# lawfuyang/ToyRenderer

Hardware: AMD Instinct MI355X
Metric: Gmeshlets/s culled (whole node), 100M meshlets (higher is better)
Workload: dtype f32

## Files before the change

### include/trhip.h

```cpp
#ifndef TRHIP_H_
#define TRHIP_H_

#include <stddef.h>
#include <stdint.h>

#ifdef __cplusplus
extern "C" {
#endif

#define TRHIP_ABI_VERSION 1

typedef struct trhip_device_t*  trhip_device;
typedef struct trhip_heap_t*    trhip_heap;
typedef struct trhip_buffer_t*  trhip_buffer;
typedef struct trhip_texture_t* trhip_texture;
typedef struct trhip_cmdlist_t* trhip_cmdlist;
typedef struct trhip_timer_t*   trhip_timer;
typedef struct trhip_pipeline_stats_t* trhip_pipeline_stats;

enum {
    TRHIP_OK = 0,
    TRHIP_ERR_INVALID = -1,
    TRHIP_ERR_HIP = -2,
    TRHIP_ERR_UNKNOWN_SHADER = -3,
    TRHIP_ERR_STATE = -4,
    TRHIP_ERR_NO_DEVICE = -5
};

enum { TRHIP_FORMAT_R16_FLOAT = 1, TRHIP_FORMAT_R32_FLOAT = 2, TRHIP_FORMAT_RG32_UINT = 3, TRHIP_FORMAT_RG16_FLOAT = 4,
       TRHIP_FORMAT_RGBA32_UINT = 5, TRHIP_FORMAT_R11G11B10_FLOAT = 6, TRHIP_FORMAT_R8_UNORM = 7, TRHIP_FORMAT_R8_UINT = 8 };

const char* trhip_last_error(void);
uint32_t    trhip_abi_version(void);
uint32_t    trhip_shader_count(void);
const char* trhip_shader_name(uint32_t index);
int         trhip_shader_exists(const char* name);

int  trhip_device_create(int device_index, trhip_device* out);
int  trhip_device_create_on_stream(int device_index, void* hip_stream, trhip_device* out);
void trhip_device_destroy(trhip_device dev);
int  trhip_device_wait_idle(trhip_device dev);
int  trhip_device_join_side_stream(trhip_device dev);
int  trhip_device_info(trhip_device dev, uint32_t* compute_units, uint32_t* wave_size, uint64_t* total_mem);
void* trhip_device_stream(trhip_device dev);

typedef struct {
    uint64_t    byteSize;
    uint32_t    structStride;
    uint32_t    canHaveUAVs;
    uint32_t    isDrawIndirectArgs;
    uint32_t    isVirtual;
    uint32_t    isVolatileConstant;
    const char* debugName;
} trhip_buffer_desc;

typedef struct {
    uint32_t    width, height, mipLevels;
    uint32_t    format;
    uint32_t    isUAV;
    uint32_t    isVirtual;
    const char* debugName;
} trhip_texture_desc;

int  trhip_heap_create(trhip_device dev, uint64_t bytes, trhip_heap* out);
void trhip_heap_release(trhip_heap heap);

int  trhip_buffer_create(trhip_device dev, const trhip_buffer_desc* desc, trhip_buffer* out);
int  trhip_buffer_wrap(trhip_device dev, void* device_ptr, const trhip_buffer_desc* desc, trhip_buffer* out);
int  trhip_buffer_memory_requirements(trhip_buffer buf, uint64_t* size, uint64_t* alignment);
int  trhip_buffer_bind_memory(trhip_buffer buf, trhip_heap heap, uint64_t offset);
void trhip_buffer_retain(trhip_buffer buf);
void trhip_buffer_release(trhip_buffer buf);
void* trhip_buffer_device_ptr(trhip_buffer buf);
uint64_t trhip_buffer_size(trhip_buffer buf);

int  trhip_texture_create(trhip_device dev, const trhip_texture_desc* desc, trhip_texture* out);
int  trhip_texture_memory_requirements(trhip_texture tex, uint64_t* size, uint64_t* alignment);
int  trhip_texture_bind_memory(trhip_texture tex, trhip_heap heap, uint64_t offset);
void trhip_texture_retain(trhip_texture tex);
void trhip_texture_release(trhip_texture tex);
void* trhip_texture_device_ptr(trhip_texture tex);
int  trhip_texture_mip_info(trhip_texture tex, uint32_t mip, uint32_t* w, uint32_t* h, uint64_t* byte_offset);
uint64_t trhip_texture_size(trhip_texture tex);

int  trhip_buffer_upload(trhip_buffer buf, uint64_t dst_offset, const void* src, uint64_t bytes);
int  trhip_buffer_download(trhip_buffer buf, uint64_t src_offset, void* dst, uint64_t bytes);
int  trhip_texture_upload(trhip_texture tex, uint32_t mip, const void* src, uint64_t bytes);
int  trhip_texture_download(trhip_texture tex, uint32_t mip, void* dst, uint64_t bytes);

int  trhip_buffer_mark_written(trhip_buffer buf);
int  trhip_texture_mark_written(trhip_texture tex);

typedef enum {
    TRHIP_BIND_CONSTANT_BUFFER = 0,
    TRHIP_BIND_PUSH_CONSTANTS  = 1,
    TRHIP_BIND_STRUCTURED_SRV  = 2,
    TRHIP_BIND_STRUCTURED_UAV  = 3,
    TRHIP_BIND_TEXTURE_SRV     = 4,
    TRHIP_BIND_TEXTURE_UAV     = 5,
    TRHIP_BIND_SAMPLER         = 6
} trhip_binding_type;

typedef struct {
    uint32_t type;
    uint32_t slot;
    void*    resource;
    uint32_t baseMip;
    uint32_t reserved;
} trhip_binding;

int  trhip_cmd_create(trhip_device dev, trhip_cmdlist* out);
void trhip_cmd_release(trhip_cmdlist cl);
int  trhip_cmd_open(trhip_cmdlist cl);
int  trhip_cmd_close(trhip_cmdlist cl);
int  trhip_cmd_write_buffer(trhip_cmdlist cl, trhip_buffer buf, uint64_t dst_offset, const void* src, uint64_t bytes);
int  trhip_cmd_clear_buffer_u32(trhip_cmdlist cl, trhip_buffer buf, uint32_t value);
int  trhip_cmd_clear_texture_f32(trhip_cmdlist cl, trhip_texture tex, float value);
int  trhip_cmd_clear_texture_u32(trhip_cmdlist cl, trhip_texture tex, uint32_t value);
int  trhip_cmd_copy_buffer(trhip_cmdlist cl, trhip_buffer dst, uint64_t dst_offset, trhip_buffer src, uint64_t src_offset, uint64_t bytes);
typedef void (*trhip_host_fn)(void* user, void* hip_stream);
int  trhip_cmd_host_callback(trhip_cmdlist cl, trhip_host_fn fn, void* user);
int  trhip_cmd_copy_texture(trhip_cmdlist cl, trhip_texture dst, trhip_texture src);
int  trhip_cmd_dispatch(trhip_cmdlist cl, const char* shader_name,
                        const trhip_binding* bindings, uint32_t num_bindings,
                        const void* push_constants, uint32_t push_bytes,
                        uint32_t gx, uint32_t gy, uint32_t gz);
int  trhip_cmd_dispatch_indirect(trhip_cmdlist cl, const char* shader_name,
                                 const trhip_binding* bindings, uint32_t num_bindings,
                                 const void* push_constants, uint32_t push_bytes,
                                 trhip_buffer args_buffer, uint32_t args_offset_bytes);
int  trhip_cmd_begin_timer(trhip_cmdlist cl, trhip_timer t);
int  trhip_cmd_end_timer(trhip_cmdlist cl, trhip_timer t);
int  trhip_cmd_begin_marker(trhip_cmdlist cl, const char* name);
int  trhip_cmd_end_marker(trhip_cmdlist cl);

int  trhip_queue_execute(trhip_device dev, const trhip_cmdlist* lists, uint32_t num_lists);

int  trhip_timer_create(trhip_device dev, trhip_timer* out);
void trhip_timer_release(trhip_timer t);
int  trhip_timer_get_ms(trhip_timer t, float* ms);

typedef struct {
    uint64_t IAVertices, IAPrimitives, VSInvocations, GSInvocations, GSPrimitives, CInvocations, CPrimitives, PSInvocations,
             HSInvocations, DSInvocations, CSInvocations, ASInvocations, MSInvocations, MSPrimitives;
} trhip_pipeline_statistics;

int  trhip_pipeline_stats_create(trhip_device dev, trhip_pipeline_stats* out);
void trhip_pipeline_stats_release(trhip_pipeline_stats q);
int  trhip_cmd_begin_pipeline_stats(trhip_cmdlist cl, trhip_pipeline_stats q);
int  trhip_cmd_end_pipeline_stats(trhip_cmdlist cl, trhip_pipeline_stats q);
int  trhip_pipeline_stats_get(trhip_pipeline_stats q, trhip_pipeline_statistics* out);

int  trhip_profile_enable(trhip_device dev, int enabled);
int  trhip_profile_filter(trhip_device dev, const char* name);
int  trhip_profile_reset(trhip_device dev);
int  trhip_profile_count(trhip_device dev, uint32_t* n);
int  trhip_profile_entry(trhip_device dev, uint32_t index, const char** name, uint64_t* launches, double* total_ms);

int  trhip_stream_create(int device_index, void** out_hip_stream);
int  trhip_stream_create_priority(int device_index, int priority_class, void** out_hip_stream);
void trhip_stream_destroy(void* hip_stream);
int  trhip_stream_synchronize(void* hip_stream);
int  trhip_event_create(int device_index, void** out_hip_event);
void trhip_event_destroy(void* hip_event);
int  trhip_event_record(void* hip_event, void* hip_stream);
int  trhip_stream_wait_event(void* hip_stream, void* hip_event);

int  trhip_launch_shard_late_info(void* hip_stream, const uint32_t* gathered_counts, uint32_t world, uint32_t rank, uint32_t* info);

#ifdef __cplusplus
}
#endif
#endif
```

### toyrenderer_amd/csrc/k_hzb.hip

```cpp
#include "cull_math.hip.h"
#include "hzb_quad.hip.h"
#include "trhip_internal.h"

using namespace interop;

namespace
{

template <bool MAX>
__global__ __launch_bounds__(256) void minMaxDownsampleKernel(const float* __restrict__ depth, uint32_t W, uint32_t H,
                                                              _Float16* __restrict__ out, uint32_t ow, uint32_t oh)
{
    const uint32_t x = blockIdx.x * 32 + (threadIdx.x & 31), y = blockIdx.y * 8 + (threadIdx.x >> 5);
    if (x >= ow || y >= oh) return;
    const float u = ((float)x + 0.5f) / (float)ow, v = ((float)y + 0.5f) / (float)oh;
    const float fx = cm::fma_(u, (float)W, -0.5f), fy = cm::fma_(v, (float)H, -0.5f);
    int x0 = (int)__builtin_floorf(fx), y0 = (int)__builtin_floorf(fy);
    int x1 = min(max(x0 + 1, 0), (int)W - 1), y1 = min(max(y0 + 1, 0), (int)H - 1);
    x0 = min(max(x0, 0), (int)W - 1);
    y0 = min(max(y0, 0), (int)H - 1);
    const float a = depth[(uint64_t)y0 * W + x0], b = depth[(uint64_t)y0 * W + x1];
    const float c = depth[(uint64_t)y1 * W + x0], d = depth[(uint64_t)y1 * W + x1];
    const float r = MAX ? cm::max_(cm::max_(a, b), cm::max_(c, d))
                        : cm::min_(cm::min_(a, b), cm::min_(c, d));
    out[(uint64_t)y * ow + x] = (_Float16)r;
}

struct SpdArgs
{
    _Float16* base;
    uint32_t width, height, mips;
    uint32_t mipOffset[16];
};

template <bool MAX>
__device__ __forceinline__ float red4(float a, float b, float c, float d)
{
    return MAX ? cm::max_(cm::max_(a, b), cm::max_(c, d)) : cm::min_(cm::min_(a, b), cm::min_(c, d));
}

template <bool MAX>
__global__ __launch_bounds__(256) void spdTileKernel(SpdArgs a, uint32_t lastMip)
{
    __shared__ float s[2][32 * 32];
    const uint32_t tid = threadIdx.x;
    const uint32_t tx = blockIdx.x, ty = blockIdx.y;
    const _Float16* m0 = a.base + a.mipOffset[0];
    {
        const uint32_t px = (tid & 15) * 2, py = (tid >> 4) * 2;
        for (uint32_t dy = 0; dy < 2; ++dy)
            for (uint32_t dx = 0; dx < 2; ++dx) {
                const uint32_t ox = px + dx, oy = py + dy;
                const uint32_t sx = tx * 64 + ox * 2, sy = ty * 64 + oy * 2;
                const float v = red4<MAX>((float)m0[(uint64_t)sy * a.width + sx], (float)m0[(uint64_t)sy * a.width + sx + 1],
                                          (float)m0[(uint64_t)(sy + 1) * a.width + sx], (float)m0[(uint64_t)(sy + 1) * a.width + sx + 1]);
                s[0][oy * 32 + ox] = v;
                if (lastMip >= 1) {
                    const uint32_t mw = a.width >> 1;
                    a.base[a.mipOffset[1] + (uint64_t)(ty * 32 + oy) * mw + tx * 32 + ox] = (_Float16)v;
                }
            }
    }
    __syncthreads();
    uint32_t cur = 0, dim = 32;
    for (uint32_t mip = 2; mip <= 6 && mip <= lastMip; ++mip) {
        const uint32_t od = dim >> 1;
        if (tid < od * od) {
            const uint32_t ox = tid % od, oy = tid / od;
            const float* p = s[cur];
            const float v = red4<MAX>(p[(2 * oy) * dim + 2 * ox], p[(2 * oy) * dim + 2 * ox + 1],
                                      p[(2 * oy + 1) * dim + 2 * ox], p[(2 * oy + 1) * dim + 2 * ox + 1]);
            s[cur ^ 1][oy * od + ox] = v;
            const uint32_t mw = a.width >> mip;
            a.base[a.mipOffset[mip] + (uint64_t)(ty * od + oy) * mw + tx * od + ox] = (_Float16)v;
        }
        __syncthreads();
        cur ^= 1;
        dim = od;
    }
}

template <bool MAX>
__global__ __launch_bounds__(256) void hzbDepthTileKernel(const float* __restrict__ depth, uint32_t W, uint32_t H, SpdArgs a, uint32_t lastMip)
{
    __shared__ float s0[64 * 64];
    __shared__ float s[2][32 * 32];
    const uint32_t tid = threadIdx.x;
    const uint32_t tx = blockIdx.x, ty = blockIdx.y;
    _Float16* m0 = a.base + a.mipOffset[0];
    const uint32_t ow = a.width, oh = a.height;
    {
        const uint32_t lx = tid & 63u, x = tx * 64 + lx;
        const float u = ((float)x + 0.5f) / (float)ow;
        const float fx = cm::fma_(u, (float)W, -0.5f);
        int x0 = (int)__builtin_floorf(fx);
        const int x1 = min(max(x0 + 1, 0), (int)W - 1);
        x0 = min(max(x0, 0), (int)W - 1);
        const int xl = min(x0, (int)W - 2);
        struct __attribute__((packed, aligned(4))) Pair { float a, b; };
        const bool wide = W >= 2u;
        Pair v0[16], v1[16];
        int rowY0, rowY1;
        {
            const uint32_t ly = (tid & 15u) * 4 + (tid >> 6), y = ty * 64 + ly;
            const float v = ((float)y + 0.5f) / (float)oh;
            const float fy = cm::fma_(v, (float)H, -0.5f);
            const int f0 = (int)__builtin_floorf(fy);
            rowY1 = min(max(f0 + 1, 0), (int)H - 1);
            rowY0 = min(max(f0, 0), (int)H - 1);
        }
#pragma unroll
        for (uint32_t it = 0; it < 16; ++it) {
            const int y0 = __builtin_amdgcn_readlane(rowY0, (int)it), y1 = __builtin_amdgcn_readlane(rowY1, (int)it);
            if (wide) {
                v0[it] = *reinterpret_cast<const Pair*>(depth + (uint64_t)y0 * W + xl);
                v1[it] = *reinterpret_cast<const Pair*>(depth + (uint64_t)y1 * W + xl);
            } else {
                v0[it] = { depth[(uint64_t)y0 * W + x0], depth[(uint64_t)y0 * W + x1] };
                v1[it] = { depth[(uint64_t)y1 * W + x0], depth[(uint64_t)y1 * W + x1] };
            }
        }
#pragma unroll
        for (uint32_t it = 0; it < 16; ++it) {
            const uint32_t ly = it * 4 + (tid >> 6), y = ty * 64 + ly;
            const float p = !wide || x0 == xl ? v0[it].a : v0[it].b, q = wide && x1 == xl ? v0[it].a : v0[it].b;
            const float r = !wide || x0 == xl ? v1[it].a : v1[it].b, t = wide && x1 == xl ? v1[it].a : v1[it].b;
            const _Float16 h = (_Float16)red4<MAX>(p, q, r, t);
            m0[(uint64_t)y * ow + x] = h;
            s0[ly * 64 + lx] = (float)h;
        }
    }
    __syncthreads();
    {
        const uint32_t px = (tid & 15) * 2, py = (tid >> 4) * 2;
        for (uint32_t dy = 0; dy < 2; ++dy)
            for (uint32_t dx = 0; dx < 2; ++dx) {
                const uint32_t ox = px + dx, oy = py + dy;
                const float v = red4<MAX>(s0[(2 * oy) * 64 + 2 * ox], s0[(2 * oy) * 64 + 2 * ox + 1],
                                          s0[(2 * oy + 1) * 64 + 2 * ox], s0[(2 * oy + 1) * 64 + 2 * ox + 1]);
                s[0][oy * 32 + ox] = v;
                if (lastMip >= 1) {
                    const uint32_t mw = a.width >> 1;
                    a.base[a.mipOffset[1] + (uint64_t)(ty * 32 + oy) * mw + tx * 32 + ox] = (_Float16)v;
                }
            }
    }
    __syncthreads();
    uint32_t cur = 0, dim = 32;
    for (uint32_t mip = 2; mip <= 6 && mip <= lastMip; ++mip) {
        const uint32_t od = dim >> 1;
        if (tid < od * od) {
            const uint32_t ox = tid % od, oy = tid / od;
            const float* p = s[cur];
            const float v = red4<MAX>(p[(2 * oy) * dim + 2 * ox], p[(2 * oy) * dim + 2 * ox + 1],
                                      p[(2 * oy + 1) * dim + 2 * ox], p[(2 * oy + 1) * dim + 2 * ox + 1]);
            s[cur ^ 1][oy * od + ox] = v;
            const uint32_t mw = a.width >> mip;
            a.base[a.mipOffset[mip] + (uint64_t)(ty * od + oy) * mw + tx * od + ox] = (_Float16)v;
        }
        __syncthreads();
        cur ^= 1;
        dim = od;
    }
}

template <bool MAX>
__global__ __launch_bounds__(256) void spdMipKernel(SpdArgs a, uint32_t mip)
{
    const uint32_t pw = (a.width >> (mip - 1)) ? (a.width >> (mip - 1)) : 1u, ph = (a.height >> (mip - 1)) ? (a.height >> (mip - 1)) : 1u;
    const uint32_t mw = (a.width >> mip) ? (a.width >> mip) : 1u, mh = (a.height >> mip) ? (a.height >> mip) : 1u;
    const uint32_t i = blockIdx.x * 256u + threadIdx.x;
    if (i >= mw * mh) return;
    const uint32_t x = i % mw, y = i / mw;
    const uint32_t x0 = min(2 * x, pw - 1), x1 = min(2 * x + 1, pw - 1);
    const uint32_t y0 = min(2 * y, ph - 1), y1 = min(2 * y + 1, ph - 1);
    const _Float16* p = a.base + a.mipOffset[mip - 1];
    a.base[a.mipOffset[mip] + i] = (_Float16)red4<MAX>((float)p[y0 * pw + x0], (float)p[y0 * pw + x1], (float)p[y1 * pw + x0], (float)p[y1 * pw + x1]);
}

struct MinMaxNote { const float* depth; uint32_t W, H; _Float16* out; uint32_t ow, oh; bool mx; };

template <bool MAX>
__global__ __launch_bounds__(1024) void spdTailKernel(SpdArgs a, uint32_t first)
{
    __shared__ float s[2][64 * 64];
    const uint32_t tid = threadIdx.x;
    uint32_t pw = (a.width >> first) ? (a.width >> first) : 1u, ph = (a.height >> first) ? (a.height >> first) : 1u;
    for (uint32_t i = tid; i < pw * ph; i += 1024) s[0][i] = (float)a.base[a.mipOffset[first] + i];
    __syncthreads();
    uint32_t cur = 0;
    for (uint32_t mip = first + 1; mip < a.mips; ++mip) {
        const uint32_t mw = (a.width >> mip) ? (a.width >> mip) : 1u, mh = (a.height >> mip) ? (a.height >> mip) : 1u;
        const float* p = s[cur];
        for (uint32_t i = tid; i < mw * mh; i += 1024) {
            const uint32_t x = i % mw, y = i / mw;
            const uint32_t x0 = min(2 * x, pw - 1), x1 = min(2 * x + 1, pw - 1);
            const uint32_t y0 = min(2 * y, ph - 1), y1 = min(2 * y + 1, ph - 1);
            const float v = red4<MAX>(p[y0 * pw + x0], p[y0 * pw + x1], p[y1 * pw + x0], p[y1 * pw + x1]);
            s[cur ^ 1][i] = v;
            a.base[a.mipOffset[mip] + i] = (_Float16)v;
        }
        __syncthreads();
        cur ^= 1;
        pw = mw; ph = mh;
    }
}

__global__ __launch_bounds__(256) void hzbQuadBuildKernel(trhip::QuadArgs a)
{
    __shared__ float s_t[9][trhip::kQuadStripCols + 1];
    trhip::hzbQuadStrip(a, blockIdx.x, s_t);
}


int recordMinMaxDownsample(trhip::DispatchCtx& ctx)
{
    const MinMaxDownsampleConsts* k = (const MinMaxDownsampleConsts*)ctx.constants(0, sizeof(MinMaxDownsampleConsts));
    TRHIP_REQUIRE(k, "%s: push constants (MinMaxDownsampleConsts, 12 bytes) missing", ctx.shaderName);
    trhip_texture_t* src = ctx.texture(TRHIP_BIND_TEXTURE_SRV, 0);
    uint32_t mip = 0;
    trhip_texture_t* dst = ctx.texture(TRHIP_BIND_TEXTURE_UAV, 0, &mip);
    TRHIP_REQUIRE(src && dst, "%s: needs Texture_SRV t0 (depth) and Texture_UAV u0 (HZB)", ctx.shaderName);
    TRHIP_REQUIRE(src->format == TRHIP_FORMAT_R32_FLOAT, "%s: depth source must be R32_FLOAT", ctx.shaderName);
    TRHIP_REQUIRE(dst->format == TRHIP_FORMAT_R16_FLOAT, "%s: HZB must be R16_FLOAT", ctx.shaderName);
    TRHIP_REQUIRE(k->m_OutputDimensions.x == dst->mipW(mip) && k->m_OutputDimensions.y == dst->mipH(mip),
                  "%s: m_OutputDimensions %ux%u does not match HZB mip %u (%ux%u)", ctx.shaderName,
                  k->m_OutputDimensions.x, k->m_OutputDimensions.y, mip, dst->mipW(mip), dst->mipH(mip));
    TRHIP_REQUIRE(!ctx.indirect, "%s: dispatched directly", ctx.shaderName);
    TRHIP_REQUIRE(ctx.gx >= (dst->mipW(mip) + 7) / 8 && ctx.gy >= (dst->mipH(mip) + 7) / 8,
                  "%s: dispatch %ux%u groups of 8x8 does not cover %ux%u (BasePassRenderers.cpp:533)", ctx.shaderName,
                  ctx.gx, ctx.gy, dst->mipW(mip), dst->mipH(mip));
    const float* depth = (const float*)src->mipPtr(0);
    _Float16* out = (_Float16*)dst->mipPtr(mip);
    const uint32_t W = src->width, H = src->height, ow = dst->mipW(mip), oh = dst->mipH(mip);
    const bool mx = k->m_bDownsampleMax != 0;
    ctx.emit("main", [=](hipStream_t s) {
        dim3 grid((ow + 31) / 32, (oh + 7) / 8);
        if (mx) TRHIP_LAUNCH(minMaxDownsampleKernel<true>, grid, dim3(256), 0, s, depth, W, H, out, ow, oh);
        else TRHIP_LAUNCH(minMaxDownsampleKernel<false>, grid, dim3(256), 0, s, depth, W, H, out, ow, oh);
        return trhip::launchStatus("minMaxDownsampleKernel"); });
    ctx.cl->peephole = { ctx.cl->ops.size() - 1, "minmaxdownsample", std::make_shared<MinMaxNote>(MinMaxNote{ depth, W, H, out, ow, oh, mx }) };
    return TRHIP_OK;
}

int recordSPD(trhip::DispatchCtx& ctx)
{
    const SPDConstants* k = (const SPDConstants*)ctx.constants(0, sizeof(SPDConstants));
    TRHIP_REQUIRE(k, "%s: push constants (SPDConstants, 32 bytes) missing", ctx.shaderName);
    uint32_t mip0 = 0;
    trhip_texture_t* tex = ctx.texture(TRHIP_BIND_TEXTURE_UAV, 2, &mip0);
    TRHIP_REQUIRE(tex, "%s: needs Texture_UAV u2 = HZB mip 0 (FFXHelpers.cpp:71)", ctx.shaderName);
    TRHIP_REQUIRE(mip0 == 0, "%s: u2 must be mip 0", ctx.shaderName);
    TRHIP_REQUIRE(tex->format == TRHIP_FORMAT_R16_FLOAT, "%s: HZB must be R16_FLOAT", ctx.shaderName);
    TRHIP_REQUIRE(k->mips == tex->mips - 1, "%s: SPDConstants.mips %u != HZB mips-1 %u (FFXHelpers.cpp:63-64)", ctx.shaderName, k->mips, tex->mips - 1);
    for (uint32_t i = 1; i < tex->mips; ++i) {
        uint32_t m = 0;
        trhip_texture_t* t = ctx.texture(TRHIP_BIND_TEXTURE_UAV, 2 + i, &m);
        TRHIP_REQUIRE(t == tex && m == i, "%s: UAV u%u must be HZB mip %u (FFXHelpers.cpp:76-81)", ctx.shaderName, 2 + i, i);
    }
    TRHIP_REQUIRE(!ctx.indirect, "%s: dispatched directly", ctx.shaderName);
    if (trhip_buffer_t* counter = ctx.buffer(TRHIP_BIND_STRUCTURED_UAV, 0)) ctx.cl->forgetUse(counter->ptr, ctx.cl->ops.size());
    const bool mx = ctx.variant == 2;
    SpdArgs a;
    memset(&a, 0, sizeof a);
    a.base = (_Float16*)tex->ptr;
    a.width = tex->width; a.height = tex->height; a.mips = tex->mips;
    for (uint32_t i = 0; i < tex->mips; ++i) a.mipOffset[i] = (uint32_t)(tex->mipOffset[i] / 2);
    if (tex->mips <= 1) return TRHIP_OK;

    uint32_t first = 0;
    const bool tiled = (tex->width % 64 == 0) && (tex->height % 64 == 0);
    const trhip_cmdlist_t::Peephole ph = ctx.cl->peephole;
    const MinMaxNote* note = (ph.kind && !strcmp(ph.kind, "minmaxdownsample") && ph.op == ctx.cl->ops.size() - 1 && ph.op != SIZE_MAX) ? (const MinMaxNote*)ph.data.get() : nullptr;
    const bool fuse = tiled && note && note->out == a.base + a.mipOffset[0] && note->ow == tex->width && note->oh == tex->height && note->mx == mx
                      && ctx.cl->ops.back().lane == 0;
    if (fuse) {
        const MinMaxNote n = *note;
        const uint32_t lastMip = tex->mips - 1 < 6 ? tex->mips - 1 : 6;
        ctx.cl->ops.pop_back();
        ctx.emit("depth_tile", [a, n, lastMip, mx](hipStream_t s) {
            dim3 grid(a.width / 64, a.height / 64);
            if (mx) TRHIP_LAUNCH(hzbDepthTileKernel<true>, grid, dim3(256), 0, s, n.depth, n.W, n.H, a, lastMip);
            else TRHIP_LAUNCH(hzbDepthTileKernel<false>, grid, dim3(256), 0, s, n.depth, n.W, n.H, a, lastMip);
            return trhip::launchStatus("hzbDepthTileKernel"); });
        first = lastMip;
    } else if (tiled) {
        const uint32_t lastMip = tex->mips - 1 < 6 ? tex->mips - 1 : 6;
        ctx.emit("tile", [a, lastMip, mx](hipStream_t s) {
            dim3 grid(a.width / 64, a.height / 64);
            if (mx) TRHIP_LAUNCH(spdTileKernel<true>, grid, dim3(256), 0, s, a, lastMip);
            else TRHIP_LAUNCH(spdTileKernel<false>, grid, dim3(256), 0, s, a, lastMip);
            return trhip::launchStatus("spdTileKernel"); });
        first = lastMip;
    }
    while ((uint64_t)tex->mipW(first) * tex->mipH(first) > 64 * 64 && first + 1 < tex->mips) {
        const uint32_t mip = first + 1;
        const uint32_t texels = tex->mipW(mip) * tex->mipH(mip);
        ctx.emit("mip", [a, mip, texels, mx](hipStream_t s) {
            if (mx) TRHIP_LAUNCH(spdMipKernel<true>, dim3((texels + 255u) / 256u), dim3(256), 0, s, a, mip);
            else TRHIP_LAUNCH(spdMipKernel<false>, dim3((texels + 255u) / 256u), dim3(256), 0, s, a, mip);
            return trhip::launchStatus("spdMipKernel"); });
        first = mip;
    }
    if (first + 1 < tex->mips) {
        ctx.emit("tail", [a, first, mx](hipStream_t s) {
            if (mx) TRHIP_LAUNCH(spdTailKernel<true>, dim3(1), dim3(1024), 0, s, a, first);
            else TRHIP_LAUNCH(spdTailKernel<false>, dim3(1), dim3(1024), 0, s, a, first);
            return trhip::launchStatus("spdTailKernel"); });
    }
    return TRHIP_OK;
}

}

namespace trhip
{

int hzbQuadEnsure(trhip_texture_t* tex)
{
    TRHIP_REQUIRE(tex && tex->ptr && tex->format == TRHIP_FORMAT_R16_FLOAT && tex->mips <= 16, "footprint-min table: needs a bound R16_FLOAT texture");
    uint64_t total = 0;
    for (uint32_t k = 0; k < tex->mips; ++k) {
        tex->quadOffset[k] = (uint32_t)total;
        total += (uint64_t)((tex->mipW(k) >> 3) + 1) * ((tex->mipH(k) >> 3) + 1) * 64u;
    }
    TRHIP_REQUIRE(total < (1ull << 31), "footprint-min table: HZB %ux%u too large", tex->width, tex->height);
    tex->quadTotal = (uint32_t)total;
    return tex->quad.allocate(tex->dev, total * 2);
}

int hzbQuadLaunchBuild(trhip_texture_t* tex, hipStream_t s)
{
    const Stamp from = { tex->version };
    if (tex->quad.current(from)) return TRHIP_OK;
    const QuadArgs a = quadArgs(tex);
    TRHIP_LAUNCH(hzbQuadBuildKernel, dim3(a.firstStrip[a.mips]), dim3(256), 0, s, a);
    tex->quad.markBuilt(from);
    return launchStatus("hzbQuadBuildKernel");
}

}

namespace
{

trhip::ShaderRegistrar r0("minmaxdownsample_CS_Main", recordMinMaxDownsample, 0);
trhip::ShaderRegistrar r1("ffx_spd_downsample_pass_CS FFX_SPD_OPTION_DOWNSAMPLE_FILTER=1", recordSPD, 1);
trhip::ShaderRegistrar r2("ffx_spd_downsample_pass_CS FFX_SPD_OPTION_DOWNSAMPLE_FILTER=2", recordSPD, 2);

}
```

### toyrenderer_amd/rhi.py

```python
from __future__ import annotations

import ctypes as C
import os

import numpy as np

_HERE = os.path.dirname(os.path.abspath(__file__))
LIB_PATH = os.environ.get("TRHIP_LIB") or os.path.join(_HERE, "lib", "libtrhip.so")

FORMAT_R16_FLOAT = 1
FORMAT_R32_FLOAT = 2
FORMAT_RG32_UINT = 3
FORMAT_RG16_FLOAT = 4
FORMAT_RGBA32_UINT = 5
FORMAT_R11G11B10_FLOAT = 6
FORMAT_R8_UNORM = 7
FORMAT_R8_UINT = 8

BIND_CONSTANT_BUFFER, BIND_PUSH_CONSTANTS, BIND_STRUCTURED_SRV, BIND_STRUCTURED_UAV, BIND_TEXTURE_SRV, BIND_TEXTURE_UAV, BIND_SAMPLER = range(7)

ABI_SYMBOLS = [
    "trhip_last_error", "trhip_abi_version", "trhip_shader_count", "trhip_shader_name", "trhip_shader_exists",
    "trhip_device_create", "trhip_device_create_on_stream", "trhip_device_destroy", "trhip_device_wait_idle",
    "trhip_device_info", "trhip_device_stream", "trhip_device_join_side_stream",
    "trhip_heap_create", "trhip_heap_release",
    "trhip_buffer_create", "trhip_buffer_wrap", "trhip_buffer_memory_requirements", "trhip_buffer_bind_memory",
    "trhip_buffer_retain", "trhip_buffer_release", "trhip_buffer_device_ptr", "trhip_buffer_size",
    "trhip_texture_create", "trhip_texture_memory_requirements", "trhip_texture_bind_memory", "trhip_texture_retain",
    "trhip_texture_release", "trhip_texture_device_ptr", "trhip_texture_mip_info", "trhip_texture_size",
    "trhip_buffer_upload", "trhip_buffer_download", "trhip_texture_upload", "trhip_texture_download",
    "trhip_buffer_mark_written", "trhip_texture_mark_written",
    "trhip_cmd_create", "trhip_cmd_release", "trhip_cmd_open", "trhip_cmd_close", "trhip_cmd_write_buffer",
    "trhip_cmd_clear_buffer_u32", "trhip_cmd_clear_texture_f32", "trhip_cmd_clear_texture_u32", "trhip_cmd_copy_buffer", "trhip_cmd_copy_texture", "trhip_cmd_host_callback", "trhip_cmd_dispatch", "trhip_cmd_dispatch_indirect",
    "trhip_cmd_begin_timer", "trhip_cmd_end_timer", "trhip_cmd_begin_marker", "trhip_cmd_end_marker",
    "trhip_queue_execute",
    "trhip_timer_create", "trhip_timer_release", "trhip_timer_get_ms",
    "trhip_pipeline_stats_create", "trhip_pipeline_stats_release", "trhip_cmd_begin_pipeline_stats",
    "trhip_cmd_end_pipeline_stats", "trhip_pipeline_stats_get",
    "trhip_profile_enable", "trhip_profile_filter", "trhip_profile_reset", "trhip_profile_count", "trhip_profile_entry",
    "trhip_launch_shard_late_info",
    "trhip_stream_create", "trhip_stream_create_priority", "trhip_stream_destroy", "trhip_stream_synchronize", "trhip_event_create", "trhip_event_destroy",
    "trhip_event_record", "trhip_stream_wait_event",
]

HOST_FN = C.CFUNCTYPE(None, C.c_void_p, C.c_void_p)


class BufferDesc(C.Structure):
    _fields_ = [("byteSize", C.c_uint64), ("structStride", C.c_uint32), ("canHaveUAVs", C.c_uint32),
                ("isDrawIndirectArgs", C.c_uint32), ("isVirtual", C.c_uint32), ("isVolatileConstant", C.c_uint32),
                ("debugName", C.c_char_p)]


class TextureDesc(C.Structure):
    _fields_ = [("width", C.c_uint32), ("height", C.c_uint32), ("mipLevels", C.c_uint32), ("format", C.c_uint32),
                ("isUAV", C.c_uint32), ("isVirtual", C.c_uint32), ("debugName", C.c_char_p)]


class Binding(C.Structure):
    _fields_ = [("type", C.c_uint32), ("slot", C.c_uint32), ("resource", C.c_void_p), ("baseMip", C.c_uint32),
                ("reserved", C.c_uint32)]


PIPELINE_STATISTICS_FIELDS = ("IAVertices", "IAPrimitives", "VSInvocations", "GSInvocations", "GSPrimitives", "CInvocations",
                              "CPrimitives", "PSInvocations", "HSInvocations", "DSInvocations", "CSInvocations", "ASInvocations",
                              "MSInvocations", "MSPrimitives")


class PipelineStatistics(C.Structure):
    _fields_ = [(f, C.c_uint64) for f in PIPELINE_STATISTICS_FIELDS]

    def as_dict(self) -> dict:
        return {f: int(getattr(self, f)) for f in PIPELINE_STATISTICS_FIELDS}


class TrhipError(RuntimeError):
    pass


_lib = None


def load() -> C.CDLL:
    global _lib
    if _lib is not None:
        return _lib
    if not os.path.exists(LIB_PATH):
        raise TrhipError(f"{LIB_PATH} is missing: build it with `python -c 'import __graft_entry__ as g; g.build()'` "
                         "(there is no CPU fallback for the HIP back end)")
    L = C.CDLL(LIB_PATH)
    vp, u32, u64, i32 = C.c_void_p, C.c_uint32, C.c_uint64, C.c_int
    L.trhip_last_error.restype = C.c_char_p
    L.trhip_abi_version.restype = u32
    L.trhip_shader_count.restype = u32
    L.trhip_shader_name.restype = C.c_char_p
    L.trhip_shader_name.argtypes = [u32]
    L.trhip_shader_exists.argtypes = [C.c_char_p]
    L.trhip_device_create.argtypes = [i32, C.POINTER(vp)]
    L.trhip_device_create_on_stream.argtypes = [i32, vp, C.POINTER(vp)]
    L.trhip_device_destroy.argtypes = [vp]
    L.trhip_device_destroy.restype = None
    L.trhip_device_wait_idle.argtypes = [vp]
    L.trhip_device_info.argtypes = [vp, C.POINTER(u32), C.POINTER(u32), C.POINTER(u64)]
    L.trhip_device_stream.argtypes = [vp]
    L.trhip_device_stream.restype = vp
    L.trhip_heap_create.argtypes = [vp, u64, C.POINTER(vp)]
    L.trhip_heap_release.argtypes = [vp]
    L.trhip_heap_release.restype = None
    L.trhip_buffer_create.argtypes = [vp, C.POINTER(BufferDesc), C.POINTER(vp)]
    L.trhip_buffer_wrap.argtypes = [vp, vp, C.POINTER(BufferDesc), C.POINTER(vp)]
    L.trhip_buffer_memory_requirements.argtypes = [vp, C.POINTER(u64), C.POINTER(u64)]
    L.trhip_buffer_bind_memory.argtypes = [vp, vp, u64]
    for n in ("trhip_buffer_retain", "trhip_buffer_release", "trhip_texture_retain", "trhip_texture_release",
              "trhip_cmd_release", "trhip_timer_release"):
        getattr(L, n).argtypes = [vp]
        getattr(L, n).restype = None
    L.trhip_buffer_device_ptr.argtypes = [vp]
    L.trhip_buffer_device_ptr.restype = vp
    L.trhip_buffer_size.argtypes = [vp]
    L.trhip_buffer_size.restype = u64
    L.trhip_texture_create.argtypes = [vp, C.POINTER(TextureDesc), C.POINTER(vp)]
    L.trhip_texture_memory_requirements.argtypes = [vp, C.POINTER(u64), C.POINTER(u64)]
    L.trhip_texture_bind_memory.argtypes = [vp, vp, u64]
    L.trhip_texture_device_ptr.argtypes = [vp]
    L.trhip_texture_device_ptr.restype = vp
    L.trhip_texture_mip_info.argtypes = [vp, u32, C.POINTER(u32), C.POINTER(u32), C.POINTER(u64)]
    L.trhip_texture_size.argtypes = [vp]
    L.trhip_texture_size.restype = u64
    L.trhip_buffer_upload.argtypes = [vp, u64, vp, u64]
    L.trhip_buffer_download.argtypes = [vp, u64, vp, u64]
    L.trhip_texture_upload.argtypes = [vp, u32, vp, u64]
    L.trhip_texture_download.argtypes = [vp, u32, vp, u64]
    L.trhip_cmd_create.argtypes = [vp, C.POINTER(vp)]
    L.trhip_cmd_open.argtypes = [vp]
    L.trhip_cmd_close.argtypes = [vp]
    L.trhip_cmd_write_buffer.argtypes = [vp, vp, u64, vp, u64]
    L.trhip_cmd_clear_buffer_u32.argtypes = [vp, vp, u32]
    L.trhip_cmd_clear_texture_f32.argtypes = [vp, vp, C.c_float]
    L.trhip_cmd_clear_texture_u32.argtypes = [vp, vp, u32]
    L.trhip_cmd_copy_buffer.argtypes = [vp, vp, u64, vp, u64, u64]
    L.trhip_cmd_copy_texture.argtypes = [vp, vp, vp]
    L.trhip_cmd_host_callback.argtypes = [vp, HOST_FN, vp]
    L.trhip_launch_shard_late_info.argtypes = [vp, vp, u32, u32, vp]
    L.trhip_stream_create.argtypes = [i32, C.POINTER(vp)]
    L.trhip_stream_create_priority.argtypes = [i32, i32, C.POINTER(vp)]
    L.trhip_stream_destroy.argtypes = [vp]
    L.trhip_stream_destroy.restype = None
    L.trhip_stream_synchronize.argtypes = [vp]
    L.trhip_event_create.argtypes = [i32, C.POINTER(vp)]
    L.trhip_event_destroy.argtypes = [vp]
    L.trhip_event_destroy.restype = None
    L.trhip_event_record.argtypes = [vp, vp]
    L.trhip_stream_wait_event.argtypes = [vp, vp]
    L.trhip_cmd_dispatch.argtypes = [vp, C.c_char_p, C.POINTER(Binding), u32, vp, u32, u32, u32, u32]
    L.trhip_cmd_dispatch_indirect.argtypes = [vp, C.c_char_p, C.POINTER(Binding), u32, vp, u32, vp, u32]
    L.trhip_cmd_begin_timer.argtypes = [vp, vp]
    L.trhip_cmd_end_timer.argtypes = [vp, vp]
    L.trhip_cmd_begin_marker.argtypes = [vp, C.c_char_p]
    L.trhip_cmd_end_marker.argtypes = [vp]
    L.trhip_queue_execute.argtypes = [vp, C.POINTER(vp), u32]
    L.trhip_timer_create.argtypes = [vp, C.POINTER(vp)]
    L.trhip_timer_get_ms.argtypes = [vp, C.POINTER(C.c_float)]
    L.trhip_pipeline_stats_create.argtypes = [vp, C.POINTER(vp)]
    L.trhip_pipeline_stats_release.argtypes = [vp]
    L.trhip_pipeline_stats_release.restype = None
    L.trhip_cmd_begin_pipeline_stats.argtypes = [vp, vp]
    L.trhip_cmd_end_pipeline_stats.argtypes = [vp, vp]
    L.trhip_pipeline_stats_get.argtypes = [vp, C.POINTER(PipelineStatistics)]
    L.trhip_profile_enable.argtypes = [vp, i32]
    L.trhip_profile_filter.argtypes = [vp, C.c_char_p]
    L.trhip_profile_reset.argtypes = [vp]
    L.trhip_buffer_mark_written.argtypes = [vp]
    L.trhip_texture_mark_written.argtypes = [vp]
    L.trhip_profile_count.argtypes = [vp, C.POINTER(u32)]
    L.trhip_profile_entry.argtypes = [vp, u32, C.POINTER(C.c_char_p), C.POINTER(u64), C.POINTER(C.c_double)]
    _lib = L
    return L


def _check(rc: int):
    if rc != 0:
        raise TrhipError(f"trhip error {rc}: {load().trhip_last_error().decode(errors='replace')}")


def shader_names():
    L = load()
    return [L.trhip_shader_name(i).decode() for i in range(L.trhip_shader_count())]


class Buffer:
    def __init__(self, dev: "Device", handle, size: int, name: str):
        self.dev, self.h, self.size, self.name = dev, handle, size, name

    def upload(self, arr: np.ndarray, offset: int = 0):
        arr = np.ascontiguousarray(arr)
        _check(load().trhip_buffer_upload(self.h, offset, arr.ctypes.data, arr.nbytes))
        return self

    def download(self, dtype=np.uint32, count: int | None = None, offset: int = 0) -> np.ndarray:
        dtype = np.dtype(dtype)
        n = (self.size - offset) // dtype.itemsize if count is None else count
        out = np.empty(n, dtype)
        if n:
            _check(load().trhip_buffer_download(self.h, offset, out.ctypes.data, out.nbytes))
        return out

    @property
    def ptr(self) -> int:
        return load().trhip_buffer_device_ptr(self.h) or 0

    def mark_written(self):
        _check(load().trhip_buffer_mark_written(self.h))

    def release(self):
        if self.h:
            load().trhip_buffer_release(self.h)
            self.h = None


class Texture:
    def __init__(self, dev: "Device", handle, w: int, h: int, mips: int, fmt: int, name: str):
        self.dev, self.h, self.w, self.hgt, self.mips, self.format, self.name = dev, handle, w, h, mips, fmt, name

    def mip_dims(self, k: int):
        return max(self.w >> k, 1), max(self.hgt >> k, 1)

    def _dtype(self):
        return {FORMAT_R16_FLOAT: np.uint16, FORMAT_RG32_UINT: np.uint64, FORMAT_RG16_FLOAT: np.float16, FORMAT_RGBA32_UINT: np.uint32,
                FORMAT_R11G11B10_FLOAT: np.uint32, FORMAT_R8_UNORM: np.uint8, FORMAT_R8_UINT: np.uint8}.get(self.format, np.float32)

    def _shape(self, mw: int, mh: int):
        return (mh, mw, 2) if self.format == FORMAT_RG16_FLOAT else (mh, mw, 4) if self.format == FORMAT_RGBA32_UINT else (mh, mw)

    def upload_mip(self, k: int, arr: np.ndarray):
        arr = np.ascontiguousarray(arr, self._dtype())
        _check(load().trhip_texture_upload(self.h, k, arr.ctypes.data, arr.nbytes))

    def download_mip(self, k: int) -> np.ndarray:
        mw, mh = self.mip_dims(k)
        out = np.empty(self._shape(mw, mh), self._dtype())
        _check(load().trhip_texture_download(self.h, k, out.ctypes.data, out.nbytes))
        return out

    def upload_chain(self, texels: np.ndarray, offsets):
        for k in range(self.mips):
            mw, mh = self.mip_dims(k)
            self.upload_mip(k, texels[offsets[k]:offsets[k] + mw * mh])

    def download_chain(self) -> np.ndarray:
        return np.concatenate([self.download_mip(k).ravel() for k in range(self.mips)])

    def mark_written(self):
        _check(load().trhip_texture_mark_written(self.h))

    def release(self):
        if self.h:
            load().trhip_texture_release(self.h)
            self.h = None


def bind(kind: int, slot: int, res=None, base_mip: int = 0) -> Binding:
    b = Binding()
    b.type, b.slot, b.baseMip = kind, slot, base_mip
    b.resource = res.h if res is not None else None
    return b


def CB(slot, buf): return bind(BIND_CONSTANT_BUFFER, slot, buf)
def PUSH(slot): return bind(BIND_PUSH_CONSTANTS, slot)
def SRV(slot, buf): return bind(BIND_STRUCTURED_SRV, slot, buf)
def UAV(slot, buf): return bind(BIND_STRUCTURED_UAV, slot, buf)
def TEX_SRV(slot, tex): return bind(BIND_TEXTURE_SRV, slot, tex)
def TEX_UAV(slot, tex, mip=0): return bind(BIND_TEXTURE_UAV, slot, tex, mip)
def SAMPLER(slot): return bind(BIND_SAMPLER, slot)


class Timer:
    def __init__(self, dev, handle):
        self.dev, self.h = dev, handle

    def ms(self) -> float:
        v = C.c_float(0)
        _check(load().trhip_timer_get_ms(self.h, C.byref(v)))
        return float(v.value)

    def release(self):
        if self.h:
            load().trhip_timer_release(self.h)
            self.h = None


class PipelineStatsQuery:
    def __init__(self, dev, handle):
        self.dev, self.h = dev, handle

    def get(self) -> dict:
        v = PipelineStatistics()
        _check(load().trhip_pipeline_stats_get(self.h, C.byref(v)))
        return v.as_dict()

    def release(self):
        if self.h:
            load().trhip_pipeline_stats_release(self.h)
            self.h = None


class CommandList:
    def __init__(self, dev: "Device", handle):
        self.dev, self.h = dev, handle
        self._keep = []
        self._keep_cb = []

    def open(self):
        self._keep.clear()
        self._keep_cb = []
        _check(load().trhip_cmd_open(self.h))
        return self

    def close(self):
        _check(load().trhip_cmd_close(self.h))
        return self

    def write_buffer(self, buf: Buffer, arr: np.ndarray, offset: int = 0):
        arr = np.ascontiguousarray(arr)
        _check(load().trhip_cmd_write_buffer(self.h, buf.h, offset, arr.ctypes.data, arr.nbytes))

    def clear_buffer_u32(self, buf: Buffer, value: int = 0):
        _check(load().trhip_cmd_clear_buffer_u32(self.h, buf.h, value))

    def clear_texture_f32(self, tex: Texture, value: float):
        _check(load().trhip_cmd_clear_texture_f32(self.h, tex.h, value))

    def clear_texture_u32(self, tex: Texture, value: int):
        _check(load().trhip_cmd_clear_texture_u32(self.h, tex.h, value))

    def copy_buffer(self, dst: Buffer, src: Buffer, nbytes: int, dst_offset: int = 0, src_offset: int = 0):
        _check(load().trhip_cmd_copy_buffer(self.h, dst.h, dst_offset, src.h, src_offset, nbytes))

    def copy_texture(self, dst: Texture, src: Texture):
        _check(load().trhip_cmd_copy_texture(self.h, dst.h, src.h))

    def constant_buffer(self, data: np.ndarray, name="cb") -> Buffer:
        data = np.ascontiguousarray(data)
        cb = self.dev.create_buffer(data.nbytes, name=name, volatile_constant=True)
        self.write_buffer(cb, data)
        self._keep.append(cb)
        return cb

    def dispatch(self, shader: str, bindings, groups, push: np.ndarray | None = None):
        arr = (Binding * len(bindings))(*bindings)
        p, pb = (None, 0) if push is None else (np.ascontiguousarray(push).ctypes.data, np.ascontiguousarray(push).nbytes)
        gx, gy, gz = groups
        _check(load().trhip_cmd_dispatch(self.h, shader.encode(), arr, len(bindings), p, pb, gx, gy, gz))

    def dispatch_indirect(self, shader: str, bindings, args: Buffer, offset: int = 0, push: np.ndarray | None = None):
        arr = (Binding * len(bindings))(*bindings)
        p, pb = (None, 0) if push is None else (np.ascontiguousarray(push).ctypes.data, np.ascontiguousarray(push).nbytes)
        _check(load().trhip_cmd_dispatch_indirect(self.h, shader.encode(), arr, len(bindings), p, pb, args.h, offset))

    def host_callback(self, fn):
        cb = HOST_FN(lambda _user, stream: fn(int(stream or 0)))
        self._keep_cb.append(cb)
        _check(load().trhip_cmd_host_callback(self.h, cb, None))

    def begin_timer(self, t: Timer): _check(load().trhip_cmd_begin_timer(self.h, t.h))
    def end_timer(self, t: Timer): _check(load().trhip_cmd_end_timer(self.h, t.h))
    def begin_pipeline_stats(self, q: PipelineStatsQuery): _check(load().trhip_cmd_begin_pipeline_stats(self.h, q.h))
    def end_pipeline_stats(self, q: PipelineStatsQuery): _check(load().trhip_cmd_end_pipeline_stats(self.h, q.h))
    def begin_marker(self, name: str): _check(load().trhip_cmd_begin_marker(self.h, name.encode()))
    def end_marker(self): _check(load().trhip_cmd_end_marker(self.h))

    def release(self):
        if self.h:
            load().trhip_cmd_release(self.h)
            self.h = None
        for b in self._keep:
            b.release()
        self._keep.clear()


class Device:
    def __init__(self, index: int = 0, stream: int | None = None, handle: int | None = None):
        L = load()
        h = C.c_void_p()
        self.owned = handle is None
        if handle is not None:
            h = C.c_void_p(handle)
        elif stream is None:
            _check(L.trhip_device_create(index, C.byref(h)))
        else:
            _check(L.trhip_device_create_on_stream(index, C.c_void_p(stream), C.byref(h)))
        self.h = h
        cu, wave, mem = C.c_uint32(), C.c_uint32(), C.c_uint64()
        _check(L.trhip_device_info(self.h, C.byref(cu), C.byref(wave), C.byref(mem)))
        self.compute_units, self.wave_size, self.total_mem = cu.value, wave.value, mem.value

    def wait_idle(self):
        _check(load().trhip_device_wait_idle(self.h))

    def create_buffer(self, nbytes: int, name="", stride=4, uav=True, indirect=False, virtual=False, volatile_constant=False) -> Buffer:
        d = BufferDesc(int(nbytes), stride, int(uav), int(indirect), int(virtual), int(volatile_constant), name.encode())
        h = C.c_void_p()
        _check(load().trhip_buffer_create(self.h, C.byref(d), C.byref(h)))
        return Buffer(self, h, int(nbytes), name)

    def wrap_buffer(self, ptr: int, nbytes: int, name="", stride=4, uav=True) -> Buffer:
        d = BufferDesc(int(nbytes), stride, int(uav), 0, 0, 0, name.encode())
        h = C.c_void_p()
        _check(load().trhip_buffer_wrap(self.h, C.c_void_p(ptr), C.byref(d), C.byref(h)))
        return Buffer(self, h, int(nbytes), name)

    def buffer_from(self, arr: np.ndarray, name="", uav=True, min_bytes: int = 4) -> Buffer:
        arr = np.ascontiguousarray(arr)
        b = self.create_buffer(max(arr.nbytes, min_bytes), name=name, stride=max(arr.dtype.itemsize, 1), uav=uav)
        if arr.nbytes:
            b.upload(arr)
        return b

    def create_texture(self, w: int, h: int, mips: int, fmt: int, name="", uav=True) -> Texture:
        d = TextureDesc(w, h, mips, fmt, int(uav), 0, name.encode())
        hd = C.c_void_p()
        _check(load().trhip_texture_create(self.h, C.byref(d), C.byref(hd)))
        return Texture(self, hd, w, h, mips, fmt, name)

    def create_command_list(self) -> CommandList:
        h = C.c_void_p()
        _check(load().trhip_cmd_create(self.h, C.byref(h)))
        return CommandList(self, h)

    def create_timer(self) -> Timer:
        h = C.c_void_p()
        _check(load().trhip_timer_create(self.h, C.byref(h)))
        return Timer(self, h)

    def create_pipeline_stats(self) -> PipelineStatsQuery:
        h = C.c_void_p()
        _check(load().trhip_pipeline_stats_create(self.h, C.byref(h)))
        return PipelineStatsQuery(self, h)

    def execute(self, *lists: CommandList):
        arr = (C.c_void_p * len(lists))(*[cl.h for cl in lists])
        _check(load().trhip_queue_execute(self.h, arr, len(lists)))

    def profile_enable(self, on: bool = True): _check(load().trhip_profile_enable(self.h, int(on)))
    def profile_reset(self): _check(load().trhip_profile_reset(self.h))
    def profile_filter(self, name: str | None): _check(load().trhip_profile_filter(self.h, name.encode() if name else None))

    def profile(self) -> dict:
        n = C.c_uint32()
        _check(load().trhip_profile_count(self.h, C.byref(n)))
        out = {}
        for i in range(n.value):
            name, cnt, ms = C.c_char_p(), C.c_uint64(), C.c_double()
            _check(load().trhip_profile_entry(self.h, i, C.byref(name), C.byref(cnt), C.byref(ms)))
            out[name.value.decode()] = (int(cnt.value), float(ms.value))
        return out

    def destroy(self):
        if self.h and self.owned:
            load().trhip_device_destroy(self.h)
        self.h = None
```

Measured before the change: 125.4.

## Stage depth bands in LDS with vectorized prefetch for HZB depth tile kernel

Adds staged variants of the HZB depth-tile kernel that cooperatively load the needed source depth rows into LDS in 16-row bands, using float4 loads when alignment allows. The next band is prefetched into registers while the current one is reduced. Mip0 and mip1 are written with packed half vectors. A host-side check picks the general path when the source footprint exceeds the staging size, and per-path launch counters are exposed for inspection. The aim is to replace scattered per-thread gathers with coalesced reuse, at the cost of extra code paths and a host-side extent scan at record time.

```diff
diff --git a/include/trhip.h b/include/trhip.h
--- a/include/trhip.h
+++ b/include/trhip.h
@@ -157,6 +157,8 @@
 int  trhip_profile_count(trhip_device dev, uint32_t* n);
 int  trhip_profile_entry(trhip_device dev, uint32_t index, const char** name, uint64_t* launches, double* total_ms);
 
+int  trhip_hzb_depth_tile_launches(uint64_t counts[3]);
+
 int  trhip_stream_create(int device_index, void** out_hip_stream);
 int  trhip_stream_create_priority(int device_index, int priority_class, void** out_hip_stream);
 void trhip_stream_destroy(void* hip_stream);
diff --git a/toyrenderer_amd/csrc/k_hzb.hip b/toyrenderer_amd/csrc/k_hzb.hip
--- a/toyrenderer_amd/csrc/k_hzb.hip
+++ b/toyrenderer_amd/csrc/k_hzb.hip
@@ -1,6 +1,9 @@
 #include "cull_math.hip.h"
 #include "hzb_quad.hip.h"
 #include "trhip_internal.h"
+
+#include <atomic>
+#include <type_traits>
 
 using namespace interop;
 
@@ -81,14 +84,145 @@
 }
 
 template <bool MAX>
+__device__ __forceinline__ void tileMips2to6(float (*s)[32 * 32], const SpdArgs& a, uint32_t tx, uint32_t ty, uint32_t tid, uint32_t lastMip)
+{
+    uint32_t cur = 0, dim = 32;
+    for (uint32_t mip = 2; mip <= 6 && mip <= lastMip; ++mip) {
+        const uint32_t od = dim >> 1;
+        if (tid < od * od) {
+            const uint32_t ox = tid % od, oy = tid / od;
+            const float* p = s[cur];
+            const float v = red4<MAX>(p[(2 * oy) * dim + 2 * ox], p[(2 * oy) * dim + 2 * ox + 1],
+                                      p[(2 * oy + 1) * dim + 2 * ox], p[(2 * oy + 1) * dim + 2 * ox + 1]);
+            s[cur ^ 1][oy * od + ox] = v;
+            const uint32_t mw = a.width >> mip;
+            a.base[a.mipOffset[mip] + (uint64_t)(ty * od + oy) * mw + tx * od + ox] = (_Float16)v;
+        }
+        __syncthreads();
+        cur ^= 1;
+        dim = od;
+    }
+}
+
+__host__ __device__ __forceinline__ int gatherFloor(uint32_t i, uint32_t outDim, uint32_t srcDim)
+{
+    const float u = ((float)i + 0.5f) / (float)outDim;
+    return (int)__builtin_floorf(__builtin_fmaf(u, (float)srcDim, -0.5f));
+}
+__host__ __device__ __forceinline__ int clampIndex(int i, uint32_t dim) { return i < 0 ? 0 : i > (int)dim - 1 ? (int)dim - 1 : i; }
+
+enum : int { kTileGeneral = 0, kTileStaged16 = 1, kTileStaged4 = 2, kTilePaths = 3 };
+constexpr uint32_t kBandRows = 16;
+constexpr uint32_t kStagePitch = 128;
+constexpr uint32_t kStageRows = 32;
+
+typedef _Float16 Half4 __attribute__((ext_vector_type(4)));
+typedef _Float16 Half2 __attribute__((ext_vector_type(2)));
+typedef float Float4 __attribute__((ext_vector_type(4)));
+
+template <typename Piece, uint32_t PASSES, uint32_t ROWS_PER_PASS>
+__device__ __forceinline__ void requestBand(Piece (&pf)[PASSES], const float* __restrict__ depth, uint32_t W, uint32_t px, uint32_t pr, int ylo, int yhi)
+{
+#pragma unroll
+    for (uint32_t k = 0; k < PASSES; ++k) {
+        const uint32_t y = min((uint32_t)ylo + k * ROWS_PER_PASS + pr, (uint32_t)yhi);
+        pf[k] = *reinterpret_cast<const Piece*>(depth + (uint64_t)y * W + px);
+    }
+}
+
+template <bool MAX, bool VEC>
+__device__ __forceinline__ void depthTileStaged(const float* __restrict__ depth, uint32_t W, uint32_t H, const SpdArgs& a, float* stage, _Float16* s0h)
+{
+    using Piece = typename std::conditional<VEC, Float4, float>::type;
+    constexpr uint32_t kPieceFloats = VEC ? 4 : 1;
+    constexpr uint32_t kPiecesPerRow = kStagePitch / kPieceFloats;
+    constexpr uint32_t kRowsPerPass = 256 / kPiecesPerRow;
+    constexpr uint32_t kPasses = kStageRows / kRowsPerPass;
+    const uint32_t tid = threadIdx.x, lane = tid & 63u;
+    const uint32_t tx = blockIdx.x, ty = blockIdx.y;
+    const uint32_t ow = a.width, oh = a.height;
+    _Float16* m0 = a.base + a.mipOffset[0];
+
+    const uint32_t col = (tid & 15u) * 4;
+    int cx0[4], cx1[4];
+#pragma unroll
+    for (uint32_t k = 0; k < 4; ++k) {
+        const int f = gatherFloor(tx * 64 + col + k, ow, W);
+        cx0[k] = clampIndex(f, W);
+        cx1[k] = clampIndex(f + 1, W);
+    }
+    const int xlo = __builtin_amdgcn_readlane(cx0[0], 0), xhi = __builtin_amdgcn_readlane(cx1[3], 15);
+    const int xa = VEC ? (xlo & ~3) : xlo;
+    const int xlast = VEC ? (xhi & ~3) : xhi;
+#pragma unroll
+    for (uint32_t k = 0; k < 4; ++k) { cx0[k] -= xa; cx1[k] -= xa; }
+    int rowY0, rowY1;
+    {
+        const int f = gatherFloor(ty * 64 + lane, oh, H);
+        rowY0 = clampIndex(f, H);
+        rowY1 = clampIndex(f + 1, H);
+    }
+    const uint32_t pr = tid / kPiecesPerRow, pc = tid % kPiecesPerRow;
+    const uint32_t px = min((uint32_t)xa + pc * kPieceFloats, (uint32_t)xlast);
+    Piece pf[kPasses];
+    requestBand<Piece, kPasses, kRowsPerPass>(pf, depth, W, px, pr, __builtin_amdgcn_readlane(rowY0, 0), __builtin_amdgcn_readlane(rowY1, kBandRows - 1));
+#pragma unroll
+    for (uint32_t b = 0; b < 64 / kBandRows; ++b) {
+        const int ylo = __builtin_amdgcn_readlane(rowY0, (int)(b * kBandRows));
+#pragma unroll
+        for (uint32_t k = 0; k < kPasses; ++k)
+            *reinterpret_cast<Piece*>(stage + (k * kRowsPerPass + pr) * kStagePitch + pc * kPieceFloats) = pf[k];
+        __syncthreads();
+        if (b + 1 < 64 / kBandRows)
+            requestBand<Piece, kPasses, kRowsPerPass>(pf, depth, W, px, pr, __builtin_amdgcn_readlane(rowY0, (int)((b + 1) * kBandRows)),
+                                                      __builtin_amdgcn_readlane(rowY1, (int)((b + 1) * kBandRows + kBandRows - 1)));
+        const uint32_t ly = b * kBandRows + (tid >> 4);
+        const float* r0 = stage + (uint32_t)(__shfl(rowY0, (int)ly) - ylo) * kStagePitch;
+        const float* r1 = stage + (uint32_t)(__shfl(rowY1, (int)ly) - ylo) * kStagePitch;
+        Half4 h;
+#pragma unroll
+        for (uint32_t k = 0; k < 4; ++k)
+            h[k] = (_Float16)red4<MAX>(r0[cx0[k]], r0[cx1[k]], r1[cx0[k]], r1[cx1[k]]);
+        *reinterpret_cast<Half4*>(m0 + (uint64_t)(ty * 64 + ly) * ow + tx * 64 + col) = h;
+        *reinterpret_cast<Half4*>(s0h + ly * 64 + col) = h;
+        __syncthreads();
+    }
+}
+
+template <bool MAX, int PATH>
 __global__ __launch_bounds__(256) void hzbDepthTileKernel(const float* __restrict__ depth, uint32_t W, uint32_t H, SpdArgs a, uint32_t lastMip)
 {
-    __shared__ float s0[64 * 64];
-    __shared__ float s[2][32 * 32];
+    __shared__ __attribute__((aligned(16))) float lds[64 * 64 + 2 * 32 * 32];
     const uint32_t tid = threadIdx.x;
     const uint32_t tx = blockIdx.x, ty = blockIdx.y;
+    const uint32_t ow = a.width, oh = a.height;
+    if constexpr (PATH != kTileGeneral) {
+        _Float16* s0h = reinterpret_cast<_Float16*>(lds + kStageRows * kStagePitch);
+        float (*s)[32 * 32] = reinterpret_cast<float (*)[32 * 32]>(lds);
+        depthTileStaged<MAX, PATH == kTileStaged16>(depth, W, H, a, lds, s0h);
+        const uint32_t px = (tid & 15) * 2, py = (tid >> 4) * 2;
+        Half4 q[4];
+#pragma unroll
+        for (uint32_t j = 0; j < 4; ++j) q[j] = *reinterpret_cast<const Half4*>(s0h + (2 * py + j) * 64 + 2 * px);
+#pragma unroll
+        for (uint32_t dy = 0; dy < 2; ++dy) {
+            Half2 o;
+#pragma unroll
+            for (uint32_t dx = 0; dx < 2; ++dx) {
+                const float v = red4<MAX>((float)q[2 * dy][2 * dx], (float)q[2 * dy][2 * dx + 1], (float)q[2 * dy + 1][2 * dx], (float)q[2 * dy + 1][2 * dx + 1]);
+                s[0][(py + dy) * 32 + px + dx] = v;
+                o[dx] = (_Float16)v;
+            }
+            if (lastMip >= 1)
+                *reinterpret_cast<Half2*>(a.base + a.mipOffset[1] + (uint64_t)(ty * 32 + py + dy) * (ow >> 1) + tx * 32 + px) = o;
+        }
+        __syncthreads();
+        tileMips2to6<MAX>(s, a, tx, ty, tid, lastMip);
+        return;
+    }
+    float* s0 = lds;
+    float (*s)[32 * 32] = reinterpret_cast<float (*)[32 * 32]>(lds + 64 * 64);
     _Float16* m0 = a.base + a.mipOffset[0];
-    const uint32_t ow = a.width, oh = a.height;
     {
         const uint32_t lx = tid & 63u, x = tx * 64 + lx;
         const float u = ((float)x + 0.5f) / (float)ow;
@@ -146,22 +280,7 @@
             }
     }
     __syncthreads();
-    uint32_t cur = 0, dim = 32;
-    for (uint32_t mip = 2; mip <= 6 && mip <= lastMip; ++mip) {
-        const uint32_t od = dim >> 1;
-        if (tid < od * od) {
-            const uint32_t ox = tid % od, oy = tid / od;
-            const float* p = s[cur];
-            const float v = red4<MAX>(p[(2 * oy) * dim + 2 * ox], p[(2 * oy) * dim + 2 * ox + 1],
-                                      p[(2 * oy + 1) * dim + 2 * ox], p[(2 * oy + 1) * dim + 2 * ox + 1]);
-            s[cur ^ 1][oy * od + ox] = v;
-            const uint32_t mw = a.width >> mip;
-            a.base[a.mipOffset[mip] + (uint64_t)(ty * od + oy) * mw + tx * od + ox] = (_Float16)v;
-        }
-        __syncthreads();
-        cur ^= 1;
-        dim = od;
-    }
+    tileMips2to6<MAX>(s, a, tx, ty, tid, lastMip);
 }
 
 template <bool MAX>
@@ -179,6 +298,37 @@
 }
 
 struct MinMaxNote { const float* depth; uint32_t W, H; _Float16* out; uint32_t ow, oh; bool mx; };
+
+uint32_t stagedExtent(uint32_t outDim, uint32_t srcDim, uint32_t step, bool align4)
+{
+    uint32_t worst = 0;
+    for (uint32_t i = 0; i < outDim; i += step) {
+        int lo = clampIndex(gatherFloor(i, outDim, srcDim), srcDim);
+        const int hi = clampIndex(gatherFloor(i + step - 1, outDim, srcDim) + 1, srcDim);
+        if (align4) lo &= ~3;
+        worst = std::max(worst, (uint32_t)(hi - lo + 1));
+    }
+    return worst;
+}
+
+int depthTilePath(const float* depth, uint32_t W, uint32_t H, uint32_t ow, uint32_t oh)
+{
+    const bool vec = W % 4 == 0 && (uintptr_t)depth % 16 == 0;
+    if (stagedExtent(ow, W, 64, vec) > kStagePitch || stagedExtent(oh, H, kBandRows, false) > kStageRows) return kTileGeneral;
+    return vec ? kTileStaged16 : kTileStaged4;
+}
+
+std::atomic<uint64_t> g_depthTileLaunches[kTilePaths];
+
+template <bool MAX>
+int launchDepthTile(int path, hipStream_t s, const float* depth, uint32_t W, uint32_t H, const SpdArgs& a, uint32_t lastMip)
+{
+    const auto kernel = path == kTileStaged16 ? hzbDepthTileKernel<MAX, kTileStaged16>
+                        : path == kTileStaged4 ? hzbDepthTileKernel<MAX, kTileStaged4> : hzbDepthTileKernel<MAX, kTileGeneral>;
+    TRHIP_LAUNCH(kernel, dim3(a.width / 64, a.height / 64), dim3(256), 0, s, depth, W, H, a, lastMip);
+    g_depthTileLaunches[path].fetch_add(1, std::memory_order_relaxed);
+    return trhip::launchStatus("hzbDepthTileKernel");
+}
 
 template <bool MAX>
 __global__ __launch_bounds__(1024) void spdTailKernel(SpdArgs a, uint32_t first)
@@ -278,11 +428,9 @@
         const MinMaxNote n = *note;
         const uint32_t lastMip = tex->mips - 1 < 6 ? tex->mips - 1 : 6;
         ctx.cl->ops.pop_back();
-        ctx.emit("depth_tile", [a, n, lastMip, mx](hipStream_t s) {
-            dim3 grid(a.width / 64, a.height / 64);
-            if (mx) TRHIP_LAUNCH(hzbDepthTileKernel<true>, grid, dim3(256), 0, s, n.depth, n.W, n.H, a, lastMip);
-            else TRHIP_LAUNCH(hzbDepthTileKernel<false>, grid, dim3(256), 0, s, n.depth, n.W, n.H, a, lastMip);
-            return trhip::launchStatus("hzbDepthTileKernel"); });
+        const int path = depthTilePath(n.depth, n.W, n.H, a.width, a.height);
+        ctx.emit("depth_tile", [a, n, lastMip, mx, path](hipStream_t s) {
+            return mx ? launchDepthTile<true>(path, s, n.depth, n.W, n.H, a, lastMip) : launchDepthTile<false>(path, s, n.depth, n.W, n.H, a, lastMip); });
         first = lastMip;
     } else if (tiled) {
         const uint32_t lastMip = tex->mips - 1 < 6 ? tex->mips - 1 : 6;
@@ -313,6 +461,13 @@
 
 }
 
+extern "C" int trhip_hzb_depth_tile_launches(uint64_t* counts)
+{
+    if (!counts) return trhip::fail(TRHIP_ERR_INVALID, "hzb_depth_tile_launches: counts is null");
+    for (int p = 0; p < kTilePaths; ++p) counts[p] = g_depthTileLaunches[p].load(std::memory_order_relaxed);
+    return TRHIP_OK;
+}
+
 namespace trhip
 {
 
diff --git a/toyrenderer_amd/rhi.py b/toyrenderer_amd/rhi.py
--- a/toyrenderer_amd/rhi.py
+++ b/toyrenderer_amd/rhi.py
@@ -38,7 +38,7 @@
     "trhip_pipeline_stats_create", "trhip_pipeline_stats_release", "trhip_cmd_begin_pipeline_stats",
     "trhip_cmd_end_pipeline_stats", "trhip_pipeline_stats_get",
     "trhip_profile_enable", "trhip_profile_filter", "trhip_profile_reset", "trhip_profile_count", "trhip_profile_entry",
-    "trhip_launch_shard_late_info",
+    "trhip_launch_shard_late_info", "trhip_hzb_depth_tile_launches",
     "trhip_stream_create", "trhip_stream_create_priority", "trhip_stream_destroy", "trhip_stream_synchronize", "trhip_event_create", "trhip_event_destroy",
     "trhip_event_record", "trhip_stream_wait_event",
 ]
@@ -142,6 +142,7 @@
     L.trhip_cmd_copy_texture.argtypes = [vp, vp, vp]
     L.trhip_cmd_host_callback.argtypes = [vp, HOST_FN, vp]
     L.trhip_launch_shard_late_info.argtypes = [vp, vp, u32, u32, vp]
+    L.trhip_hzb_depth_tile_launches.argtypes = [C.POINTER(u64)]
     L.trhip_stream_create.argtypes = [i32, C.POINTER(vp)]
     L.trhip_stream_create_priority.argtypes = [i32, i32, C.POINTER(vp)]
     L.trhip_stream_destroy.argtypes = [vp]
@@ -188,6 +189,12 @@
     return [L.trhip_shader_name(i).decode() for i in range(L.trhip_shader_count())]
 
 
+def hzb_depth_tile_launches() -> dict:
+    counts = (C.c_uint64 * 3)()
+    _check(load().trhip_hzb_depth_tile_launches(counts))
+    return {"general": int(counts[0]), "staged16": int(counts[1]), "staged4": int(counts[2])}
+
+
 class Buffer:
     def __init__(self, dev: "Device", handle, size: int, name: str):
         self.dev, self.h, self.size, self.name = dev, handle, size, name
```

New measurement: 123.1. -1.9%, worse.
